# pgriewank/SAMSIM

Hardware: AMD Instinct MI355X
Metric: column-timesteps/sec (higher is better)
Workload: dtype f64

## Files before the change

samsim_amd/csrc/samsim_kernels.hip:

```cpp
#include <hip/hip_runtime.h>
#include <math.h>

#include <type_traits>

#include "samsim_device.h"
#include "samsim_probe.h"
#include "samsim_step_types.h"
#include "samsim_thermo.h"
#include "samsim_surface.h"
#include "samsim_sweeps_fused.h"
#include "samsim_melt.h"
#include "samsim_sweeps_unfused.h"
#include "samsim_regrid.h"
#include "samsim_tracers.h"

namespace {

template <class K>
__device__ RARE void vital_signs(Col &c, const Ctx &x) {
  const samsim_config &g = x.p->cfg;
  const int Na = c.Na;
  double sH = 0.0, sm = 0.0, sS = 0.0, resist = 0.0, sth = 0.0, sS1 = 0.0, sm1 = 0.0;
  for (int k = 1; k <= Na; ++k) {
    const double H_abs = LAY(SAMSIM_A_H_ABS, k), m = LAY(SAMSIM_A_M, k), S_abs = LAY(SAMSIM_A_S_ABS, k);
// ... 96 lines not shown
    if (time > 86400.0 * 25.0) CL(T2m) = 15.0;
    else if (time > 86400.0 * 15.0) CL(T2m) = 1.0;
  } else if (K::general && CFG(testcase) == 9) {
    if (time < 19.75 * 3600.0) CL(T2m) = 0.0;
    else if (time < 86400.0 * 3.0 + 2.25 * 3600.0) CL(T2m) = -15.0;
    else CL(T2m) = 1.0;
  } else if (K::general && CFG(testcase) == 34) {
    if (time < 2.0 * 3600.0) CL(T2m) = 0.0;
    else if (time < 86400.0 * 5.0) CL(T2m) = -15.0;
    else if (time < 86400.0 * 7.0) CL(T2m) = -5.0;
    else CL(T2m) = 1.0;
  } else if (K::general && CFG(testcase) == 6) {
    const double t[8] = {1714.0, 1676.0, 1525.0, 1483.0, 1385.0, 1349.0, 1160.0, 1100.0};
    for (int i = 0; i < 8; ++i) {
      if (time > t[i] * 60.0) { CL(T2m) = (i == 0) ? -19.0 : ((i & 1) ? -5.0 : -18.0); break; }
    }
  }
}

template <class K>
__device__ __forceinline__ void column_step(Col &c, Ctx &x, long long col, double time, int tc, bool out_step, bool next_out,
                                            bool last_step) {
  const samsim_config &g = x.p->cfg;
  const int N = c.N;

  if (out_step) {
    vital_signs<K>(c, x);
    if ((c.flags & COLF_RESTART) && col >= x.out_col0 && col < x.out_col0 + x.out_ncols) {
      const size_t oc = (size_t)(col - x.out_col0), on = (size_t)x.out_ncols;
      for (int k = 1; k <= N; ++k) x.out_lay[((size_t)SAMSIM_A_RAY * N + (k - 1)) * on + oc] = LAY(SAMSIM_A_RAY, k);
    }
  }

  if (CFG(atmoflux_flag) == 2) {
    if (time == time_input(tc)) {
      CL(T2m) = x.f_T2m[x.soff + tc - 1];
      CL(liquid_precip) = x.f_precip[x.soff + tc - 1];
    } else {
      const double temp = (time - time_input(tc - 1)) / (time_input(tc) - time_input(tc - 1));
      CL(T2m) = (1.0 - temp) * x.f_T2m[x.soff + tc - 2] + temp * x.f_T2m[x.soff + tc - 1];
      CL(liquid_precip) = (1.0 - temp) * x.f_precip[x.soff + tc - 2] + temp * x.f_precip[x.soff + tc - 1];
    }
    CL(T2m) = CL(T2m) + GSI(SAMSIM_S_DT2M);
    CL(liquid_precip) = CL(liquid_precip) * GSI(SAMSIM_S_PRECIP_SCALE);
  }

  c.bgc_flood = 0.0; c.bgc_grav = false;
  snow_fall<K>(c, x);
  snow_block<K>(c, x);
  if (c.status) return;

  c.ray_all = (c.flags & COLF_DIRTY) != 0;
  const bool whole_wave = !wave_any(!c.ray_all);
  if (c.ray_all) { ST_COUNT(CT_DIRTY, 1); ST_COUNT(CT_L_DIRTY, (unsigned long long)__popcll(__ballot(1))); sweep_thermo_expulsion<K>(c, x, out_step, whole_wave); }
  else prologue_top_layer<K>(c, x);
  c.flags &= (COLF_REGULAR | COLF_FLUSHED);
  if (c.status) return;

  int Na = c.Na;
  const bool do_grav = (CFG(grav_flag) == 2 && Na > 1), do_beer = (CFG(boundflux_flag) == 2);
  const bool coupling = (CL(m_snow) > 0.0 && CL(thick_snow) < g.thick_min);
  const bool flood_possible = (CFG(flood_flag) > 1 && CL(m_snow) > 0.0 && CFG(freeboard_snow_flag) == 0 &&
                               CL(m_snow) > c.buoy_s * (rho_l - rho_s));
  [[maybe_unused]] const bool fused_col = do_grav && !out_step && (c.step + 1 != 1) && (!flood_possible || (CFG(flood_flag) == 2 && !coupling)) &&
                     !(K::general && CFG(testcase) == 5 && c.step + 1 == 2) && !HAS_BGC &&
                     !(K::general && CFG(prescribe_flag) == 2)
                     && (c.flags & COLF_REGULAR) != 0
      ;
#if SAMSIM_PATH_MODE == 1
  const bool fused = false;
#else
  const bool fused = !wave_any(!fused_col);
#endif

  ST_MARK(ST_PRO);
  ST_COUNT(CT_WAVESTEPS, 1);
  ST_COUNT(CT_LANES, (unsigned long long)__popcll(__ballot(1)));
  ST_COUNT(CT_L_COUPLING, (unsigned long long)__popcll(__ballot(coupling)));
  ST_COUNT(CT_L_FLOODP, (unsigned long long)__popcll(__ballot(flood_possible)));
  ST_COUNT(CT_L_IRREG, (unsigned long long)__popcll(__ballot((c.flags & COLF_REGULAR) == 0)));
  ST_COUNT(CT_L_UNFUSED, (unsigned long long)__popcll(__ballot(!fused_col)));
  bool surface_done = false;
  if (fused) {
    ST_COUNT(CT_FUSED, 1);
    if (flood_possible) {
      ExpelledEnds en;
      sweep_expulsion_transfer<K, true>(c, x, &en);
      THICK_RULE_INIT(tr);
      if (en.psi_gN > 0.0) {
        const double temp2 = en.psi_gN * THICK_AT(tr, Na) * rho_l;
        en.mN = en.mN + temp2;
        en.SN = en.SN + temp2 * x.S_bu_bottom;
        en.HN = en.HN + temp2 * c_l * g.T_bottom;
      }
      const double buoy = c.buoy_s * (rho_l - rho_s) + en.buoy_g * rho_l;
      if (CL(m_snow) > buoy) {
        GS(FREEBOARD) = (buoy - CL(m_snow)) / rho_l;
        if (GS(FREEBOARD) < 0.0) {
          FloodEnds e;
          e.S1 = en.S1; e.H1 = en.H1; e.m1 = en.m1; e.th1 = LAY(SAMSIM_A_THICK, 1);
          e.SN = en.SN; e.HN = en.HN; e.mN = en.mN; e.TN = en.TN;
          const double th1_before = e.th1;
          flood_core<K>(c, x, SPEC(SP_FL_HP), SPEC(SP_FL_SALL), e);
          LAY(SAMSIM_A_THICK, 1) = e.th1;
          refresh_ray_top<K>(c, x, e.th1, en.psi_l1, en.S_br1);
          c.flags |= COLF_FLOODED;
          SPEC(SP_FLD_S1) = e.S1; SPEC(SP_FLD_H1) = e.H1; SPEC(SP_FLD_M1) = e.m1; SPEC(SP_FLD_TH1_BEFORE) = th1_before;
          if (e.deep) { c.flags |= COLF_FLOOD_DEEP; SPEC(SP_FL_HP) = e.incS; SPEC(SP_FL_SALL) = e.incH; }
        }
      }
    }
    testcase_scalars<K>(c, x, g, time);
    const bool late_rad = wave_any(coupling);
    double beer0 = 0.0;
    if (!late_rad) {
      beer0 = radiation_header<K>(c, x, time, tc);
      c.frad = 0.0;
    }
    bool store_default = true, decide_psi = false;
    if (K::fixed && K::boundflux_flag == 2 && K::flush_flag == 5) { store_default = next_out || last_step; decide_psi = true; }
    if (K::fixed && K::flush_flag == 1) store_default = next_out || last_step;
    if (do_beer && !late_rad) sweep_beer<K>(c, x, beer0);
    sweep_down_fused<K>(c, x, store_default, decide_psi, surface_done, coupling, late_rad, time, tc, do_beer);
    ST_MARK(ST_DFUSED);
    if (c.status) return;
  } else {
    ST_COUNT(CT_UNFUSED, 1);
    c.psi_full = true;
    down_unfused<K>(c, x, col, time, tc, out_step, coupling, do_grav, do_beer);
    ST_MARK(ST_DUNFUSED);
    if (c.status) return;
  }

  if (K::general && CFG(tank_flag) == 2) {
    double sS = 0.0, sm = 0.0;
    for (int k = 1; k <= c.Na; ++k) { sS += LAY(SAMSIM_A_S_ABS, k); sm += LAY(SAMSIM_A_M, k); }
    x.S_bu_bottom = (g.S_total - sS) / (g.m_total - sm);
    if (HAS_BGC) {
      double sb = 0.0;
      for (int k = 1; k <= c.Na; ++k) sb += BGC(0, k);
      const double v = (x.bgc_total0 - sb) / (g.m_total - sm);
      for (int t = 0; t < x.n_bgc; ++t) BGC_BOT(t) = v;
    }
  }

  if (!surface_done) surface_flux<K>(c, x);
  ST_MARK(ST_SURF);
  sweep_up_fused<K>(c, x, col, next_out, next_out || last_step);
  ST_MARK(ST_UP);
  if (c.status) return;

  const double melt_thick_snow_old = CL(melt_thick_snow);
  snow_block<K>(c, x);
  if (c.status) return;
  CL(melt_thick_snow) = melt_thick_snow_old + CL(melt_thick_snow);

  bool fb_valid = false;
  if (Na > 1 && CFG(flush_flag) > 2 && (CFG(boundflux_flag) == 2 || (K::general && CFG(boundflux_flag) == 3))) {
    const bool lab = K::general && CFG(boundflux_flag) == 3;
    const double T_surf = lab ? CL(T2m) : CL(T_top);
    const double T_freeze = func_T_freeze(quot(LAY(SAMSIM_A_S_ABS, 1), LAY(SAMSIM_A_M, 1)), CFG(salt_flag), x.tf_c3);
    GS(T_FREEZE) = T_freeze;
    CL(melt_thick) = 0.0;
    const double psi_s1 = LAY(SAMSIM_A_PSI_S, 1);
    if (psi_s1 < psi_s_top_min || T_surf >= T_freeze) {
      if (!c.psi_full) refill_psi_rows<K>(c, x);
      ST_COUNT(CT_L_FREEBOARD, (unsigned long long)__popcll(__ballot(1)));
      GS(FREEBOARD) = func_freeboard<K>(c, x);
      fb_valid = true;
      if (GS(FREEBOARD) > 0.0000000000001) {
        double thick1 = LAY(SAMSIM_A_THICK, 1);
        const double thick1_in = thick1;
        double melt_thick = 0.0;
        sub_melt_thick(LAY(SAMSIM_A_PSI_L, 1), psi_s1, LAY(SAMSIM_A_PSI_G, 1), LAY(SAMSIM_A_T, 1), T_freeze, T_surf, CL(fl_Q1),
                       CL(thick_snow), g.dt, melt_thick, thick1, g.thick_min);
        CL(melt_thick) = melt_thick;
        if (lab) CL(melt_thick) = dmax(CL(melt_thick), 0.0);
        if (CL(thick_snow) >= g.thick_min / 100.0 && CL(melt_thick) > 0.00000000001 && CL(melt_thick_snow) == 0.0) {
          double H_abs = LAY(SAMSIM_A_H_ABS, 1), m = LAY(SAMSIM_A_M, 1);
          const double shift = 1.0 / dmax(GS(PSI_G_SNOW), 0.01) * CL(melt_thick);
          if (shift >= CL(thick_snow)) {
            CL(melt_thick) = CL(melt_thick) - CL(thick_snow) * GS(PSI_G_SNOW);
            H_abs = H_abs + CL(H_abs_snow);
            m = m + CL(m_snow);
// ... 253 lines not shown
```

samsim_amd/csrc/samsim_surface.h:

```cpp
#ifndef SAMSIM_SURFACE_H
#define SAMSIM_SURFACE_H

namespace {

template <class K>
__device__ RARE int snow_coupling_core(Col &c, const Ctx &x, double &H_abs, const double m, const double S_bu, double &T, double &phi) {
  const Salt &s = x.salt;
  double H;
  const double m_snow = CL(m_snow), S_abs_snow = GS(S_ABS_SNOW);
  double phi_sn = GS(PHI_S);
  int rc = 0;
  H_abs = H_abs + m_snow * latent_heat + CL(H_abs_snow);
  CL(H_abs_snow) = -m_snow * latent_heat;
  H = H_abs / m;
#define COUPLE_GETT()                                                                                      \
  do {                                                                                                     \
    double hs = CL(H_abs_snow) / m_snow;                                                                     \
    double T_sn = CL(T_snow);                                                                              \
    rc |= getT(s, hs, S_abs_snow / m_snow, hs / c_l, T_sn, phi_sn);                                        \
    CL(T_snow) = T_sn;                                                                                     \
    rc |= getT(s, H, S_bu, H / c_l, T, phi);                                                               \
  } while (0)
  COUPLE_GETT();
  if (T > 0.0 && H_abs <= -CL(H_abs_snow)) {
// ... 174 lines not shown
      const double temp = (time - time_input(tc - 1)) / (time_input(tc) - time_input(tc - 1));
      CL(fl_sw) = (1.0 - temp) * x.f_sw[x.soff + tc - 2] + temp * x.f_sw[x.soff + tc - 1];
      CL(fl_lw) = (1.0 - temp) * x.f_lw[x.soff + tc - 2] + temp * x.f_lw[x.soff + tc - 1];
    }
  } else if (CFG(atmoflux_flag) == 1) {
    double day = (time + 86400.0 * 180.0) / 86400.0;
    while (day > 360.0) day = day - 360.0;
    const double a = (day - 164.0) / (double)47.9f, b = (day - 206.0) / (double)53.1f;
    CL(fl_sw) = 314.0 * exp(-0.5 * (a * a));
    if (day < 60.0 || day > 300.0) CL(fl_sw) = 0.0;
    GSI(SAMSIM_S_FL_REST) = 118.0 * exp(-0.5 * (b * b)) + 179.0;
  }
  const double pen = (CL(thick_snow) < g.thick_min) ? penetr : 0.0;
  return pen * (1.0 - CL(albedo)) * CL(fl_sw);
}

__device__ __forceinline__ double radiative_T_top(const Col &c, double fl_rest, double T1, double thick_min) {
  double T_old = (CL(thick_snow) < thick_min) ? T1 : CL(T_snow);
  const double emi = (CL(thick_snow) < thick_min) ? emissivity_ice : emissivity_snow;
  const double pen = (CL(thick_snow) < thick_min) ? penetr : 0.0;
  T_old = T_old + zeroK;
  double temp1 = (1.0 - CL(albedo)) * (1.0 - pen) * CL(fl_sw) + fl_rest;
  temp1 = temp1 + emi * 3.0 * sigma * pow_4(T_old);
  temp1 = quot(temp1, emi * 4.0 * sigma * (T_old * T_old * T_old));
  temp1 = temp1 - zeroK;
  T_old = temp1 + zeroK;
  temp1 = (1.0 - CL(albedo)) * (1.0 - pen) * CL(fl_sw) + fl_rest;
  temp1 = temp1 + emi * 3.0 * sigma * pow_4(T_old);
  temp1 = quot(temp1, emi * 4.0 * sigma * (T_old * T_old * T_old));
  temp1 = temp1 - zeroK;
  return temp1;
}

template <class K>
__device__ __forceinline__ void surface_flux(Col &c, const Ctx &x) {
  const samsim_config &g = x.p->cfg;
  const int Na = c.Na;
  const double psi_s1 = LAY(SAMSIM_A_PSI_S, 1), psi_l1 = LAY(SAMSIM_A_PSI_L, 1), psi_g1 = LAY(SAMSIM_A_PSI_G, 1);
  const double thick1 = LAY(SAMSIM_A_THICK, 1), T1 = LAY(SAMSIM_A_T, 1);
  const double k1 = psi_s1 * k_s + psi_l1 * k_l + psi_g1 * 0.0;
  if (CFG(boundflux_flag) == 1) {
    double fl = (T1 - CL(T_top)) / (thick1 / (2.0 * k1));
    if (fabs(fl) > g.max_flux_plate) fl = fl / fabs(fl) * g.max_flux_plate;
    CL(fl_Q1) = fl;
    return;
  }
  if (K::general && CFG(boundflux_flag) == 3) {
    GS(T_FREEZE) = dmin(func_T_freeze(LAY(SAMSIM_A_S_ABS, Na) / LAY(SAMSIM_A_M, Na), CFG(salt_flag), x.tf_c3), 0.0);
    CL(T_top) = T1;
    CL(fl_Q1) = g.alpha_flux_instable * (CL(T_top) - CL(T2m));
    if (CL(fl_Q1) < 0.0) {
      CL(T_top) = dmax(GS(T_FREEZE), T1);
      CL(fl_Q1) = g.alpha_flux_stable * (CL(T_top) - CL(T2m));
    }
    return;
  }
  const double thick_min = g.thick_min;
  const double fl_rest = (!K::general || CFG(atmoflux_flag) == 2) ? CL(fl_lw) + 0.0 + 0.0 : GSI(SAMSIM_S_FL_REST);
  const double emi = (CL(thick_snow) < thick_min) ? emissivity_ice : emissivity_snow;
  const double pen = (CL(thick_snow) < thick_min) ? penetr : 0.0;
  double temp1;
  CL(T_top) = radiative_T_top(c, fl_rest, T1, thick_min);

  double Tf;
  if (CL(thick_snow) >= thick_min / 100.0) Tf = 0.0;
  else Tf = func_T_freeze(quot(LAY(SAMSIM_A_S_ABS, 1), LAY(SAMSIM_A_M, 1)), CFG(salt_flag), x.tf_c3);

  GS(T_FREEZE) = Tf;

  const double k_snow = (CL(thick_snow) >= thick_min / 100.0) ? func_k_snow(CL(m_snow), CL(thick_snow)) : 0.0;
  const double flq_snow_ice = quot(T1 - CL(T_snow), quot(CL(thick_snow), 2.0 * k_snow) + quot(thick1, 2.0 * (psi_s1 * k_s + psi_l1 * k_l)));
  if (CL(T_top) > Tf && Na > 1) {
    temp1 = emi * sigma * pow_4(Tf + zeroK) - (1.0 - CL(albedo)) * (1.0 - pen) * CL(fl_sw) - fl_rest;
    if (CL(thick_snow) >= thick_min) { CL(fl_Q_snow) = temp1; CL(fl_Q1) = flq_snow_ice; }
    else if (CL(thick_snow) >= thick_min / 100.0) { CL(fl_Q_snow) = temp1; CL(fl_Q1) = 0.0; }
    else CL(fl_Q1) = temp1;
    CL(T_top) = Tf;
  } else {
    if (CL(thick_snow) >= thick_min) {
      CL(fl_Q1) = flq_snow_ice;
      CL(fl_Q_snow) = quot(CL(T_snow) - CL(T_top), quot(CL(thick_snow), 2.0 * k_snow));
    } else if (CL(thick_snow) > thick_min / 100.0 && CL(thick_snow) < thick_min) {
      CL(fl_Q1) = 0.0;
      double k = CL(thick_snow) / (CL(thick_snow) + thick1) * k_snow + thick1 / (CL(thick_snow) + thick1) * k1;
      CL(fl_Q_snow) = (CL(T_snow) - CL(T_top)) / ((CL(thick_snow) + thick1) / (2.0 * k));
    } else {
      CL(fl_Q1) = (T1 - CL(T_top)) / (thick1 / (2.0 * k1));
    }
  }
}

__device__ __forceinline__ void sub_melt_thick(double psi_l, double psi_s, double psi_g, double T, double T_freeze, double T_top, double fl_Q,
                               double thick_snow, double dt, double &melt_thick, double &thick, double thick_min) {
  melt_thick = 0.0;
  if (thick_snow < thick_min && T_top >= T_freeze) {
    melt_thick = -fl_Q - 2.0 * (psi_l * k_l + psi_s * k_s) / thick * (T_freeze - T);
    melt_thick = melt_thick * dt / dmax(latent_heat * rho_s * psi_s, 0.000000000000001);
    melt_thick = dmin(psi_l * thick, melt_thick);
  }
  if (psi_s < psi_s_top_min) melt_thick = thick * (1.0 - psi_s / psi_s_top_min);
  if (melt_thick > 0.0 && psi_g > gas_snow_ice2) {
    if (melt_thick > (psi_g - gas_snow_ice2) * thick) {
      melt_thick = melt_thick - (psi_g - gas_snow_ice2) * thick;
      thick = thick * (1.0 - (psi_g - gas_snow_ice2));
    } else {
      thick = thick - melt_thick;
      melt_thick = 0.0;
    }
  }
}

}

#endif
```

samsim_amd/csrc/samsim_sweeps_fused.h:

```cpp
#ifndef SAMSIM_SWEEPS_FUSED_H
#define SAMSIM_SWEEPS_FUSED_H

namespace {


struct RayScan {
  double minp, stp, st;
  double bot, botterm, perm_bot, S_br_bot;
  double buoy_s, min_psi_s;
};
__device__ __forceinline__ void ray_scan_init(RayScan &r) {
  r.minp = 1.0e300; r.stp = 0.0; r.st = 0.0; r.bot = 0.0; r.botterm = 0.0; r.perm_bot = 0.0; r.S_br_bot = 0.0;
  r.buoy_s = 0.0; r.min_psi_s = 1.0e300;
}

struct Expelled { double psi_s, psi_l, psi_g, V_ex; };
__device__ __forceinline__ Expelled expulsion(double phi, double thick, double m, double rth) {
  Expelled e;
  const double V_s = m * phi * (1.0 / rho_s), V_l = m * (1.0 - phi) * (1.0 / rho_l);
  e.V_ex = dmax(V_l + V_s - thick, 0.0);
  e.psi_s = V_s * rth;
  e.psi_l = (V_l - e.V_ex) * rth;
  e.psi_g = (thick - V_l - V_s + e.V_ex) * rth;
  e.psi_l = dmax(e.psi_l, 0.0);
  e.psi_g = dmax(e.psi_g, 0.0);
  return e;
}

template <class K>
__device__ __forceinline__ void s1_layer(Col &c, const Ctx &x, int k, int Na, bool do_ray, double T, double phi, double S_bu,
                                         double m, double thick, double rth, RayScan &r, bool sparse_rows = false, const double *S_br_T = nullptr) {
  const samsim_config &g = x.p->cfg;
  const double S_br = S_br_T ? *S_br_T : S_br_clamped(x.salt, T, S_bu);
  const Expelled e = expulsion(phi, thick, m, rth);
  r.min_psi_s = dmin(r.min_psi_s, e.psi_s);
  r.buoy_s += e.psi_s * thick;
  if (k == 1) c.psi_l_top = e.psi_l;
  if (do_ray) {
    const double perm = x.p17 * pow_3p1(1000.0 * fabs(e.psi_l));
    if (k == Na) {
      r.S_br_bot = S_br;
      r.bot = thick * e.psi_s / psi_s_min;
      r.perm_bot = perm;
      r.botterm = r.bot / perm;
    } else {
      const double height = r.st + r.bot;
      r.minp = dmin(r.minp, perm);
      r.stp = r.stp + quot(thick, perm);
      r.st = r.st + thick;
      double ray;
      const double d_S_br = S_br - r.S_br_bot;
      const bool harmonic = CFG(harmonic_flag) == 2;
      const double h_sum = harmonic ? r.st + r.bot : 0.0, h_den = harmonic ? r.stp + r.botterm : 0.0;
      if (sparse_rows && harmonic && k != 1 && !x.ray_rows_all) {
        constexpr double q_ray = ray_crit * (1.0 - 0x1p-20) * (kappa_l * mu);
        const double P = grav_f * rho_l * bbeta * d_S_br * height * h_sum, Q = q_ray * h_den;
        ST_COUNT(CT_RAY_ROWS, 1);
        if ((__builtin_amdgcn_ballot_w64(!(P < Q)) & __builtin_amdgcn_ballot_w64(!(r.minp < x.p14))) == 0ull) {
          ST_COUNT(CT_RAY_ROWS_BOUND, 1);
          return;
        }
      }
      if (harmonic) {
        const double hp = (r.minp < x.p14) ? 0.0 : quot(h_sum, h_den);
        ray = grav_f * rho_l * bbeta * d_S_br * height * hp;
      } else {
        ray = grav_f * rho_l * bbeta * d_S_br * height * dmin(r.minp, r.perm_bot);
      }
      ray = ray * (1.0 / (kappa_l * mu));
      ray = dmax(ray, 0.0);
      if (!sparse_rows) {
        LAYU(SAMSIM_A_RAY, k) = ray;
      } else if (k == 1 || x.ray_rows_all || wave_any(ray > ray_crit)) {
        LAYU(SAMSIM_A_RAY, k) = ray;
        x.rflag[(k - 1) >> 6] = x.rflag[(k - 1) >> 6] | (1ull << ((k - 1) & 63));
      }
    }
  }
}

template <class K>
__device__ __forceinline__ void flood_handover(Col &c, const Ctx &x, const RayScan &all, const RayScan &below_top, double thick_bottom) {
  const samsim_config &g = x.p->cfg;
  if (!(CFG(flood_flag) > 1 && c.Na > 1 && CL(m_snow) > all.buoy_s * (rho_l - rho_s))) return;
  SPEC(SP_FL_HP) = quot(all.st + all.bot, all.stp + all.botterm);
  SPEC(SP_FL_SALL) = all.st + thick_bottom;
  SPEC(SP_MINP) = below_top.minp; SPEC(SP_STP) = below_top.stp; SPEC(SP_ST) = below_top.st;
  SPEC(SP_BOT) = below_top.bot; SPEC(SP_BOTTERM) = below_top.botterm; SPEC(SP_SBR_BOT) = below_top.S_br_bot;
}

template <class K>
__device__ __forceinline__ void prologue_top_layer(Col &c, const Ctx &x) {
  const samsim_config &g = x.p->cfg;
  const int Na = c.Na;
  const bool do_ray = (CFG(grav_flag) >= 2 && Na > 1);
  RayScan r;
  r.minp = SPEC(SP_MINP); r.stp = SPEC(SP_STP); r.st = SPEC(SP_ST);
  r.bot = SPEC(SP_BOT); r.botterm = SPEC(SP_BOTTERM); r.perm_bot = SPEC(SP_PERM_BOT);
  r.S_br_bot = SPEC(SP_SBR_BOT); r.buoy_s = SPEC(SP_BUOY_S); r.min_psi_s = SPEC(SP_MIN_PSI_S);
  const RayScan r_below_top = r;
  const double H_abs = LAY(SAMSIM_A_H_ABS, 1), m = LAY(SAMSIM_A_M, 1), thick = LAY(SAMSIM_A_THICK, 1);
  double S_abs = LAY(SAMSIM_A_S_ABS, 1);
  if (S_abs < 0.0) { S_abs = 0.0; LAY(SAMSIM_A_S_ABS, 1) = S_abs; }
  double S_bu, H;
  per_mass(S_abs, H_abs, m, S_bu, H);
  if (K::general && CFG(prescribe_flag) == 2) LAY(SAMSIM_A_S_BU, 1) = S_abs / m;
  const double T_test = (Na > 1) ? LAY(SAMSIM_A_T, 2) : g.T_bottom;
  double T, phi = 0.0;
  const int rc = getT_chain(x.salt, H, S_bu, T_test, T, phi);
  LAY(SAMSIM_A_T, 1) = T;
  LAY(SAMSIM_A_PHI, 1) = phi;
  s1_layer<K>(c, x, 1, Na, do_ray, T, phi, S_bu, m, thick, recip(thick), r);
  if (do_ray && CFG(flood_flag) > 1 && CL(m_snow) > r.buoy_s * (rho_l - rho_s)) {
    THICK_RULE_INIT(tr);
    flood_handover<K>(c, x, r, r_below_top, THICK_AT(tr, Na));
  }
  c.neg_psi = r.min_psi_s < 0.0;
  c.buoy_s = r.buoy_s;
  if (rc) STOPC(rc, 1);
}

template <class K>
__device__ RARE void sweep_beer(Col &c, const Ctx &x, double beer0) {
  const samsim_config &g = x.p->cfg;
  const int Na = c.Na;
  if (!wave_any(beer0 != 0.0)) { c.frad = 0.0; return; }
  if ((c.flags & COLF_REGULAR) != 0) {
    const int n0 = __builtin_amdgcn_readfirstlane(Na);
    const bool same = !wave_any(Na != n0);
    const int kend = same ? n0 : wave_max(Na);
    const int b0 = g.n_top, b1 = g.n_top + g.n_middle;
    double temp2 = beer0, frad = 0.0;
#pragma unroll 1
    for (int st = 0; st < 4; ++st) {
      const int klo = st == 0 ? 1 : (st == 1 ? 2 : (st == 2 ? b0 + 1 : b1 + 1));
      const int khi_s = st == 0 ? 1 : (st == 1 ? b0 : (st == 2 ? b1 : kend));
      if (klo > kend) break;
      if (klo > khi_s) continue;
      const int khi = khi_s < kend ? khi_s : kend;
      const double thick = st == 0 ? LAYU(SAMSIM_A_THICK, 1) : (st == 2 ? LAYU(SAMSIM_A_THICK, g.n_top + 1) : g.thick_0);
      const double e = exp(-extinc * thick);
      if (same) {
        const int kmul = khi < kend ? khi : kend - 1;
        for (int k = klo; k <= kmul; ++k) temp2 = temp2 * e;
        if (khi == kend) frad = temp2 - temp2 * e;
// ... 6 lines not shown
      }
    }
    c.frad = frad;
  } else {
    double temp2 = beer0, e = 0.0, th_prev = -1.0;
    for (int k = 1; k <= Na; ++k) {
      const double thick = LAYU(SAMSIM_A_THICK, k);
      if (thick != th_prev) { e = exp(-extinc * thick); th_prev = thick; }
      if (k == Na) c.frad = temp2 - temp2 * e;
      temp2 = temp2 * e;
    }
  }
}

__device__ __forceinline__ double heat_conductance(double psi_s, double psi_l, double rth) {
  return (2.0 * (psi_s * k_s + psi_l * k_l)) * rth;
}
__device__ __forceinline__ double heat_flux_between(double dT, double g_a, double g_b) {
  return quot(dT * (g_a * g_b), g_a + g_b);
}

__device__ __forceinline__ double out_of_row(double v) {
#if defined(__HIP_DEVICE_COMPILE__)
  double r;
  asm volatile("v_mov_b64 %0, %1" : "=v"(r) : "v"(v));
  return r;
#else
  return v;
#endif
}

template <class K>
__device__ __forceinline__ void sweep_down_fused(Col &c, const Ctx &x, bool store_default, bool decide_psi, bool &surface_done,
                                                 bool couple, bool late_rad, double time, int tc, bool do_beer) {
  const samsim_config &g = x.p->cfg;
  const Salt &s = x.salt;
  const int Na = c.Na;
  const double dt = g.dt;
  double heat_loss = 0.0, cum = 0.0, sum_before = 0.0, sum_after = 0.0, minS = 1.0e300;
  double fb_a2 = 0.0, fb_g2 = 0.0;
  int stop_layer = 0;
  bool store_psi = true;
  double g_up = 0.0, flq_up = 0.0;
  double esum = 0.0;

  struct Ld { double T, S_abs, m, H_abs, ray; };
  struct Raw { double T, S_abs, m, S_bu, S_br, H_abs, ray, H; };
  auto load_ld = [&](int j) -> Ld {
    Ld r;
    r.T = LAYU_LD(SAMSIM_A_T, j);
    r.S_abs = LAYU_LD(SAMSIM_A_S_ABS, j);
    r.m = LAYU_LD(SAMSIM_A_M, j);
    r.H_abs = LAYU_LD(SAMSIM_A_H_ABS, j);
    r.ray = (j <= Na - 1 && ray_row_valid(c, x, j)) ? LAYU(SAMSIM_A_RAY, j) : 0.0;
    return r;
  };
  auto finish = [&](const Ld &l, int j) -> Raw {
    Raw r;
    r.T = l.T; r.S_abs = l.S_abs; r.m = l.m; r.H_abs = l.H_abs; r.ray = l.ray;
    per_mass(r.S_abs, r.H_abs, r.m, r.S_bu, r.H);
    r.S_br = S_br_clamped(s, r.T, r.S_bu);
    return r;
  };
  auto S_br_below = [&](const Ld &l) -> double {
    double S_bu, H;
    per_mass(l.S_abs, l.H_abs, l.m, S_bu, H);
    return S_br_clamped(s, l.T, S_bu);
  };
  struct Lay { double T, SA, mA, S_abs, H_abs, m, flup; bool ch; };

  double flm_j = 0.0;
  double T_up = 0.0, S_br_up = 0.0, S_abs_up = 0.0;
  const int N = c.N;
  Raw raw = finish(load_ld(1), 1);
  Ld ahead = load_ld(2), ahead2 = ahead;
  Lay prev = {0, 0, 1, 0, 0, 0, 0, true};
  double flup_pp = 0.0;
  auto layer = [&](const int j, const Ld &below, const double thick, const double rth, auto last_tag, auto first_tag) {
    constexpr bool LAST = decltype(last_tag)::value, FIRST = decltype(first_tag)::value;
    if (!LAST && !FIRST) { ISA_MARK("D_LAYER_A"); }
    double H_abs = raw.H_abs;
    const Expelled ex = expulsion(phi_from_T(s, raw.H, raw.S_bu, raw.S_br), thick, raw.m, rth);
    const double V_ex = ex.V_ex;
    double psi_g = ex.psi_g, m = raw.m, S_abs = raw.S_abs;
    const double T = raw.T, S_br = raw.S_br;
    double flm_next;
    if (j == 1 || psi_g < (double)0.001f) {
      flm_next = (j == 1) ? -V_ex * rho_l : -V_ex * rho_l + flm_j;
    } else {
      flm_next = -dmax((V_ex - psi_g * thick) * rho_l, 0.0);
      psi_g = dmax(quot(psi_g * thick - V_ex, thick), 0.0);
    }
    if (!FIRST) { fb_a2 += ex.psi_s * thick; fb_g2 += psi_g * thick; }
    if (store_psi || j == 1) {
      LAYU(SAMSIM_A_PSI_S, j) = ex.psi_s;
      LAYU(SAMSIM_A_PSI_L, j) = ex.psi_l;
      LAYU(SAMSIM_A_PSI_G, j) = psi_g;
    }
    const bool flooded_here = FIRST && (c.flags & COLF_FLOODED) != 0;
    const double th_l = flooded_here ? LAYU(SAMSIM_A_THICK, 1) : thick;
    const double gj = heat_conductance(ex.psi_s, ex.psi_l, flooded_here ? recip(th_l) : rth);
    const double flq = (j >= 2) ? heat_flux_between(T - prev.T, g_up, gj) : 0.0;
    if (j == 2) c.flq2 = flq;
    m = m + flm_next - flm_j;
    if (flm_next < 0.0) {
      H_abs = H_abs + flm_next * T * c_l;
      S_abs = S_abs + dmax(flm_next * S_br, -S_abs);
    }
    if (flm_j < 0.0) {
      H_abs = H_abs - flm_j * T_up * c_l;
      S_abs = S_abs - dmax(flm_j * S_br_up, -S_abs_up);
    }
    bool ch = LAST || (flm_next < 0.0) || (flm_j < 0.0);
#if SAMSIM_STAMPS == 2
    if (!LAST && !FIRST) {
      ST_COUNT(CT_ROWS, 1);
      if (__ballot(flm_next < 0.0 || flm_j < 0.0) == 0ull) ST_COUNT(CT_ROWS_STILL, 1);
    }
#endif
    const double SA = S_abs, mA = m;
    S_br_up = S_br;
    flm_j = flm_next;
    double Tl = T;
    if (FIRST && couple) {
      double phi1 = LAYU(SAMSIM_A_PHI, 1);
      const double S_bu1 = S_abs / m;
      LAYU(SAMSIM_A_S_BU, 1) = S_bu1;
      const int rcc = snow_coupling_core<K>(c, x, H_abs, m, S_bu1, Tl, phi1);
      LAYU(SAMSIM_A_T, 1) = Tl;
      LAYU(SAMSIM_A_PHI, 1) = phi1;
      if (rcc && !c.status) { c.status = rcc; x.err_step[c.col] = c.step + 1; x.err_layer[c.col] = 1; }
    }
    if (flooded_here) {
      S_abs = SPEC(SP_FLD_S1); H_abs = SPEC(SP_FLD_H1); m = SPEC(SP_FLD_M1);
      ch = true;
      c.flags &= ~COLF_FLOODED;
    }
    if (LAST) {
      if (psi_g > 0.0) {
        const double t2 = psi_g * thick * rho_l;
        m = m + t2;
        S_abs = S_abs + t2 * x.S_bu_bottom;
        H_abs = H_abs + t2 * c_l * g.T_bottom;
      }
      if (c.flags & COLF_FLOOD_DEEP) {
        S_abs = S_abs + SPEC(SP_FL_HP);
        H_abs = H_abs + SPEC(SP_FL_SALL);
        c.flags &= ~COLF_FLOOD_DEEP;
      }
      if (CFG(turb_flag) == 2) {
        const double turb = Turb_A * exp(Turb_B * (-ocean_density<K>(x) + func_density(T, quot(S_abs, m)))) * dt;
        S_abs = S_abs - turb * (S_abs / m - x.S_bu_bottom);
      }
    }
    if (!LAST && !FIRST) { ISA_MARK("D_LAYER_B"); }
    ST_MARK(ST_D_A);
    sum_before += S_abs;
    double flup = cum;
    if (!LAST) {
      const double ray = raw.ray;
      if (ray > ray_crit && S_br > S_br_below(below)) {
        const double psi_s = ex.psi_s;
        if (psi_s > 0.001 && (flooded_here ? quot(S_abs, m) : quot(SA, mA)) > 0.1) {
          ST_COUNT(CT_DRAIN_WAVE, 1);
          ST_COUNT(CT_DRAIN_LANE, (unsigned long long)__popcll(__ballot(1)));
          const double psi_l = ex.psi_l;
          double flux = x_grav * (ray - ray_crit) * dt * th_l;
          flux = dmin(flux, psi_l * rho_l * th_l);
          S_abs = S_abs - flux * S_br;
          if (S_abs < 0.0 && !stop_layer) stop_layer = j;
// ... 3 lines not shown
          cum = cum + flux;
          flup = dmin(cum, psi_l * rho_l * th_l);
          ch = true;
        }
      }
    }
    sum_after += S_abs;
#if defined(__HIP_DEVICE_COMPILE__)
    asm volatile("" : "+v"(sum_before), "+v"(sum_after));
#endif
    if (!LAST && !FIRST) { ISA_MARK("D_LAYER_C"); }
    if (j > 1) {
      if (prev.flup > 0.0) {
        prev.H_abs = prev.H_abs + prev.flup * T * c_l;
        prev.S_abs = prev.S_abs + dmin(prev.flup * S_br_clamped(s, T, quot(SA, mA)), S_abs);
        prev.ch = true;
      }
      if (flup_pp > 0.0) {
        prev.H_abs = prev.H_abs - flup_pp * prev.T * c_l;
        prev.S_abs = prev.S_abs - dmin(flup_pp * S_br_clamped(s, prev.T, quot(prev.SA, prev.mA)), prev.S_abs);
        prev.ch = true;
      }
      if (j - 1 >= 2) {
        const double H_b = prev.H_abs;
        prev.H_abs = prev.H_abs + (flq - flq_up) * dt;
        prev.H_abs = prev.H_abs + c.frad * dt;
        esum += H_b - prev.H_abs;
      }
      if (wave_any(prev.ch)) {
        LAYU(SAMSIM_A_M, j - 1) = prev.m;
        LAYU(SAMSIM_A_S_ABS, j - 1) = prev.S_abs;
      }
      LAYU(SAMSIM_A_H_ABS, j - 1) = prev.H_abs;
      minS = dmin(minS, prev.S_abs);
      flup_pp = prev.flup;
    }
    g_up = gj; flq_up = flq;
    T_up = out_of_row(T); S_abs_up = out_of_row(SA);
    prev.T = FIRST ? out_of_row(Tl) : T_up; prev.SA = S_abs_up; prev.mA = mA; prev.S_abs = out_of_row(S_abs); prev.H_abs = out_of_row(H_abs);
    prev.m = m; prev.flup = flup; prev.ch = ch;
    if (!LAST && !FIRST) { ISA_MARK("D_LAYER_END"); }
    ST_MARK(ST_D_B);
  };
  const int jmax = wave_max(Na);
  auto request = [&](const int j) { ahead2 = load_ld(j + 2 <= N ? j + 2 : N); };
  auto advance = [&](const int j) { raw = finish(ahead, j + 1); ahead = ahead2; };
  const double thick1 = (c.flags & COLF_FLOODED) ? SPEC(SP_FLD_TH1_BEFORE) : LAYU(SAMSIM_A_THICK, 1);
  if (1 < Na) { request(1); layer(1, ahead, thick1, recip(thick1), std::false_type{}, std::true_type{}); advance(1); }
  if (2 < Na) { request(2); layer(2, ahead, g.thick_0, recip(g.thick_0), std::false_type{}, std::false_type{}); advance(2); }
  if (late_rad) {
    const double beer0 = radiation_header<K>(c, x, time, tc);
    c.frad = 0.0;
    if (do_beer) sweep_beer<K>(c, x, beer0);
  }
  if (decide_psi && Na >= 3) {
    surface_flux<K>(c, x);
    surface_done = true;
    const double thick_min = g.thick_min;
    const double Tf = func_T_freeze(quot(LAYU(SAMSIM_A_S_ABS, 1), LAYU(SAMSIM_A_M, 1)), CFG(salt_flag), x.tf_c3);
    bool snow_wet = false;
    if (CL(thick_snow) > 0.0) {
      const double H_new = CL(H_abs_snow) + (CL(fl_Q1) - CL(fl_Q_snow)) * dt;
      snow_wet = !(CL(thick_snow) >= thick_min) || !(H_new / CL(m_snow) <= -latent_heat);
    }
    store_psi = store_default || LAYU(SAMSIM_A_PSI_S, 1) < psi_s_top_min || CL(T_top) >= Tf || snow_wet || CL(melt_thick_snow) > 0.0;
  } else {
    store_psi = store_default || decide_psi;
  }
  c.psi_full = store_psi;
  {
    const int b0 = g.n_top, b1 = g.n_top + g.n_middle;
    Ld ahead3 = ahead;
    auto single = [&](const int j, const double th_s, const double rth_s) {
      ahead2 = load_ld(j + 2 <= N ? j + 2 : N);
      layer(j, ahead, th_s, rth_s, std::false_type{}, std::false_type{});
      raw = finish(ahead, j + 1);
      ahead = ahead2;
    };
    int j = 3;
    for (int stretch = 0; stretch < 3; ++stretch) {
      const int hi_s = stretch == 0 ? b0 : (stretch == 1 ? b1 : N);
      const int hi = hi_s < jmax - 1 ? hi_s : jmax - 1;
      const double th_s = stretch == 1 ? LAYU(SAMSIM_A_THICK, g.n_top + 1) : g.thick_0, rth_s = recip(th_s);
      for (; j + 2 <= hi; j += 3) {
        ISA_MARK("D_ITER_BEGIN");
        ST_MARK(ST_DFUSED);
        if (j + 2 < Na) {
          ST_COUNT(CT_DOWN_TRIPS, 3);
          ahead2 = load_ld(j + 2 <= N ? j + 2 : N);
          layer(j, ahead, th_s, rth_s, std::false_type{}, std::false_type{});
          raw = finish(ahead, j + 1);
          ahead3 = load_ld(j + 3 <= N ? j + 3 : N);
          layer(j + 1, ahead2, th_s, rth_s, std::false_type{}, std::false_type{});
          raw = finish(ahead2, j + 2);
          ahead = load_ld(j + 4 <= N ? j + 4 : N);
          layer(j + 2, ahead3, th_s, rth_s, std::false_type{}, std::false_type{});
          raw = finish(ahead3, j + 3);
        } else if (j < Na) {
          ISA_MARK("D_RARE_BEGIN");
          ST_COUNT(CT_DOWN_TRIPS, 1);
          single(j, th_s, rth_s);
          if (j + 1 < Na) { ST_COUNT(CT_DOWN_TRIPS, 1); single(j + 1, th_s, rth_s); }
        }
        ISA_MARK("D_ITER_END");
      }
      for (; j <= hi; ++j) {
        if (j < Na) single(j, th_s, rth_s);
      }
    }
  }
  const double thick_Na = (Na > g.n_top && Na <= g.n_top + g.n_middle) ? LAYU(SAMSIM_A_THICK, g.n_top + 1) : g.thick_0;
  layer(Na, ahead, thick_Na, recip(thick_Na), std::true_type{}, std::false_type{});
  if (prev.flup > 0.0) {
    prev.H_abs = prev.H_abs + prev.flup * g.T_bottom * c_l;
    prev.S_abs = prev.S_abs + dmin(prev.flup * S_br_clamped(s, g.T_bottom, x.S_bu_bottom), x.S_bu_bottom * 2000.0);
  }
  if (flup_pp > 0.0) {
    prev.H_abs = prev.H_abs - flup_pp * prev.T * c_l;
    prev.S_abs = prev.S_abs - dmin(flup_pp * S_br_clamped(s, prev.T, quot(prev.SA, prev.mA)), prev.S_abs);
  }
  CL(grav_drain) = CL(grav_drain) + prev.flup;
  if (CFG(grav_heat_flag) == 2) prev.H_abs = prev.H_abs + heat_loss - prev.flup * c_l * g.T_bottom;
  {
    const double H_b = prev.H_abs;
    prev.H_abs = prev.H_abs + (c.fl_q_bottom - flq_up) * dt;
    prev.H_abs = prev.H_abs + c.frad * dt;
    c.esum = esum + (H_b - prev.H_abs);
  }
  LAYU(SAMSIM_A_M, Na) = prev.m;
  LAYU(SAMSIM_A_S_ABS, Na) = prev.S_abs;
  LAYU(SAMSIM_A_H_ABS, Na) = prev.H_abs;
  minS = dmin(minS, prev.S_abs);
  if (store_psi) { SPEC(SP_FB_A2) = fb_a2; SPEC(SP_FB_G2) = fb_g2; }
  CL(grav_salt) = CL(grav_salt) + sum_before;
  CL(grav_salt) = CL(grav_salt) - sum_after;
  if (stop_layer) STOPC(21234, stop_layer);
  if (minS < 0.0) STOPC(1337, 0);
}

template <class K>
__device__ __forceinline__ void sweep_up_fused(Col &c, const Ctx &x, long long col, bool next_is_output, bool store_phi) {
  const samsim_config &g = x.p->cfg;
  const Salt &s = x.salt;
  const int Na = c.Na;
  const double dt = g.dt, thick_min = g.thick_min;
  const bool thin_snow = (CL(thick_snow) >= thick_min / 100.0 && CL(thick_snow) < thick_min);
  const bool do_ray = (CFG(grav_flag) >= 2 && Na > 1);
  const bool keep_ray = next_is_output && col >= x.out_col0 && col < x.out_col0 + x.out_ncols;
  const double H_abs_snow_before = CL(H_abs_snow);
  double esum = c.esum;
  double T_test = g.T_bottom;
  int rc = 0, rc_layer = 0;
  RayScan r;
  ray_scan_init(r);
  if (keep_ray) {
    const size_t oc = (size_t)(col - x.out_col0), on = (size_t)x.out_ncols;
    for (int k = 1; k <= c.N - 1; ++k) x.out_lay[((size_t)SAMSIM_A_RAY * c.N + (k - 1)) * on + oc] = LAYU(SAMSIM_A_RAY, k);
  }
  for (int w = 0; w <= (c.N - 1) >> 6; ++w) x.rflag[w] = 0ull;
  __builtin_amdgcn_wave_barrier();
  if (do_ray && Na <= c.N - 1 && x.ray_rows_all) LAYU(SAMSIM_A_RAY, Na) = 0.0;
  struct UL { double th, H, m, S; };
  const bool regular_wave = !wave_any((c.flags & COLF_REGULAR) == 0);
  UL cur, nxt, nn;
  bool alive = true, neg_salt = false;
  NewtonConsts nc_s = newton_consts(s);
  auto body = [&](const int k, const UL &row, const double th_k, const double rth_k, auto top_tag, auto lite_tag) {
    constexpr bool TOP = decltype(top_tag)::value;
    constexpr bool LITE = decltype(lite_tag)::value;
    const double H_k = row.H, m_k = row.m, S_k = row.S;
    double H_abs = H_k;
    const double m = m_k;
    if (TOP) {
      const double flq_below = (Na >= 2) ? c.flq2 : c.fl_q_bottom;
// ... 25 lines not shown
      if (!TOP) { ST_COUNT(CT_ABOVE_ROWS, 1); if (__ballot(evals < 0)) ST_COUNT(CT_ABOVE_FAST, 1); }
      evals &= 0x7fffffff;
      const bool was_odd = (evals >> 30) & 1;
      const int redo = (evals >> 16) & 0x3fff;
      evals &= 0xffff;
      const unsigned long long om = __ballot(was_odd);
      if (om) { ST_COUNT(CT_ODD_LANES, (unsigned long long)__popcll(om)); ST_COUNT(CT_ODD_WAVES, 1); ST_COUNT(CT_ODD_EVALS_WAVE, (unsigned long long)wave_max(redo)); }
    }
    ST_COUNT(CT_UP_TRIPS, 1);
    ST_COUNT(CT_NEWTON_WAVE, (unsigned long long)wave_max(evals));
    { int tot = 0; unsigned long long mk = __ballot(1); while (mk) { const int ln = __ffsll((long long)mk) - 1; tot += __builtin_amdgcn_readlane(evals, ln); mk &= mk - 1; }
      ST_COUNT(CT_NEWTON_LANE, (unsigned long long)tot); }
#else
    int rr = TOP ? getT(s, H, S_bu, T_test, T, phi) : getT_chain<LITE>(s, H, S_bu, T_test, T, phi, nullptr, LITE ? nullptr : &S_br_T, &nc_s);
#endif
    if (!TOP) { ISA_MARK("U_GETT_END"); }
    ST_MARK(ST_U_GETT);
    if (rr && !rc) { rc = rr; rc_layer = k; }
    T_test = T;
    LAYU(SAMSIM_A_T, k) = T;
    if (store_phi || TOP || k >= Na - 1) LAYU(SAMSIM_A_PHI, k) = phi;
    if (!TOP && !LITE) {
      neg_salt = neg_salt || (S_abs < 0.0);
      s1_layer<K>(c, x, k, Na, do_ray, T, phi, S_bu, m, th_k, rth_k, r, true, &S_br_T);
    }
    ST_MARK(ST_U_TAIL);
  };
  const int kmax = wave_max(Na);
  auto load3 = [&](int j) -> UL { UL u; u.th = 0.0; u.H = LAYU_LD(SAMSIM_A_H_ABS, j); u.m = LAYU_LD(SAMSIM_A_M, j); u.S = LAYU_LD(SAMSIM_A_S_ABS, j); return u; };
  auto load4 = [&](int j) -> UL { UL u = load3(j); u.th = LAYU(SAMSIM_A_THICK, j); return u; };
  auto layers = [&](auto lite_tag) {
  if (regular_wave) {
    const int kc = kmax >= 2 ? kmax - 1 : 1;
    UL a = load3(kmax), b = load3(kc), d = b;
    auto one = [&](const int k, const UL &row, UL &req, const double th_s, const double rth_s) {
      req = load3(k >= 3 ? k - 2 : 1);
      if (k <= Na) body(k, row, th_s, rth_s, std::false_type{}, lite_tag);
    };
    const int b0 = g.n_top, b1 = g.n_top + g.n_middle;
    int k = kmax;
    for (int stretch = 0; stretch < 3; ++stretch) {
      const int klo = stretch == 0 ? b1 + 1 : (stretch == 1 ? b0 + 1 : 2);
      const double th_s = stretch == 1 ? LAYU(SAMSIM_A_THICK, g.n_top + 1) : g.thick_0, rth_s = recip(th_s);
      nc_s = newton_consts(s);
      for (; k - 2 >= klo; k -= 3) {
        ISA_MARK("U_ITER_BEGIN");
        ST_MARK(ST_UP);
        one(k, a, d, th_s, rth_s);
        ISA_MARK("U_LAYER_2");
        one(k - 1, b, a, th_s, rth_s);
        ISA_MARK("U_LAYER_3");
        one(k - 2, d, b, th_s, rth_s);
        ISA_MARK("U_ITER_END");
      }
      for (; k >= klo; --k) {
        ISA_MARK("U_REST_BEGIN");
        ST_MARK(ST_UP);
        one(k, a, d, th_s, rth_s);
        a = b; b = d;
        ISA_MARK("U_REST_END");
      }
    }
    cur = a;
  } else {
    cur = load4(Na); nxt = load4(Na >= 2 ? Na - 1 : 1); nn = nxt;
    for (int k = kmax; k >= 2; --k) {
      if (k > Na) continue;
      nn = load4(k >= 3 ? k - 2 : 1);
      body(k, cur, cur.th, recip(cur.th), std::false_type{}, lite_tag);
      cur = nxt; nxt = nn;
    }
  }
  };
  const bool lite = K::fixed && CFG(flush_flag) == 5 && wave_any((c.flags & COLF_FLUSHED) != 0);
  if (lite) { ST_COUNT(CT_LITE, 1); layers(std::true_type{}); } else layers(std::false_type{});
  __builtin_amdgcn_wave_barrier();
  if (neg_salt || lite) c.flags |= COLF_DIRTY;
  body(1, cur, LAYU(SAMSIM_A_THICK, 1), 0.0, std::true_type{}, std::false_type{});
  if (!alive) return;
  if (!lite) {
  SPEC(SP_MINP) = r.minp; SPEC(SP_STP) = r.stp; SPEC(SP_ST) = r.st;
  SPEC(SP_BOT) = r.bot; SPEC(SP_BOTTERM) = r.botterm; SPEC(SP_PERM_BOT) = r.perm_bot;
  SPEC(SP_SBR_BOT) = r.S_br_bot; SPEC(SP_BUOY_S) = r.buoy_s; SPEC(SP_MIN_PSI_S) = r.min_psi_s;
  }
  double bal = esum + (H_abs_snow_before - CL(H_abs_snow));
  bal = bal + (double)Na * (c.frad * dt);
  if (thin_snow || CL(thick_snow) >= thick_min) bal = bal + c.fl_q_bottom * dt - CL(fl_Q_snow) * dt;
  else bal = bal + c.fl_q_bottom * dt - CL(fl_Q1) * dt;
  if (fabs(bal / dt) > 0.00001) STOPC(431, 0);
  if (rc) STOPC(rc, rc_layer);
}

}

#endif
```

Baseline: 778.8 million.

## Hand off top and bottom layer values in registers between prologue and sweeps

The top-layer prologue values (T, S, m, H, thickness, ray) are passed into the fused down-sweep in registers, and the layer-1 porosity and temperature are captured during the down-sweep to feed a new surface_flux_core. The down-sweep's final bottom rows are handed to the up-sweep so it can skip reloading them. This removes redundant global-memory reloads of layer data across stages. In exchange it adds register pressure and several correctness-sensitive conditions (flooded flag, kc mismatch, wave uniformity).

```diff
diff --git a/samsim_amd/csrc/samsim_kernels.hip b/samsim_amd/csrc/samsim_kernels.hip
--- a/samsim_amd/csrc/samsim_kernels.hip
+++ b/samsim_amd/csrc/samsim_kernels.hip
@@ -152,6 +152,7 @@
     }
   }
 
+  ISA_MARK("P_HEAD");
   if (CFG(atmoflux_flag) == 2) {
     if (time == time_input(tc)) {
       CL(T2m) = x.f_T2m[x.soff + tc - 1];
@@ -166,14 +167,18 @@
   }
 
   c.bgc_flood = 0.0; c.bgc_grav = false;
+  ISA_MARK("P_SNOW");
   snow_fall<K>(c, x);
   snow_block<K>(c, x);
   if (c.status) return;
 
+  ISA_MARK("P_PROLOGUE");
   c.ray_all = (c.flags & COLF_DIRTY) != 0;
   const bool whole_wave = !wave_any(!c.ray_all);
+  const bool top_handed = !wave_any(c.ray_all);
+  TopHand top = {0.0, 0.0, 0.0, 0.0, 0.0, 0.0};
   if (c.ray_all) { ST_COUNT(CT_DIRTY, 1); ST_COUNT(CT_L_DIRTY, (unsigned long long)__popcll(__ballot(1))); sweep_thermo_expulsion<K>(c, x, out_step, whole_wave); }
-  else prologue_top_layer<K>(c, x);
+  else prologue_top_layer<K>(c, x, top);
   c.flags &= (COLF_REGULAR | COLF_FLUSHED);
   if (c.status) return;
 
@@ -201,6 +206,7 @@
   ST_COUNT(CT_L_IRREG, (unsigned long long)__popcll(__ballot((c.flags & COLF_REGULAR) == 0)));
   ST_COUNT(CT_L_UNFUSED, (unsigned long long)__popcll(__ballot(!fused_col)));
   bool surface_done = false;
+  BottomHand bot = {0.0, 0.0, 0.0, 0.0, 0.0, 0.0, 0};
   if (fused) {
     ST_COUNT(CT_FUSED, 1);
     if (flood_possible) {
@@ -241,7 +247,7 @@
     if (K::fixed && K::boundflux_flag == 2 && K::flush_flag == 5) { store_default = next_out || last_step; decide_psi = true; }
     if (K::fixed && K::flush_flag == 1) store_default = next_out || last_step;
     if (do_beer && !late_rad) sweep_beer<K>(c, x, beer0);
-    sweep_down_fused<K>(c, x, store_default, decide_psi, surface_done, coupling, late_rad, time, tc, do_beer);
+    sweep_down_fused<K>(c, x, store_default, decide_psi, surface_done, coupling, late_rad, time, tc, do_beer, top_handed, top, bot);
     ST_MARK(ST_DFUSED);
     if (c.status) return;
   } else {
@@ -266,10 +272,12 @@
 
   if (!surface_done) surface_flux<K>(c, x);
   ST_MARK(ST_SURF);
-  sweep_up_fused<K>(c, x, col, next_out, next_out || last_step);
+  ISA_MARK("P_UP_ENTRY");
+  sweep_up_fused<K>(c, x, col, next_out, next_out || last_step, fused, bot);
   ST_MARK(ST_UP);
   if (c.status) return;
 
+  ISA_MARK("P_POST");
   const double melt_thick_snow_old = CL(melt_thick_snow);
   snow_block<K>(c, x);
   if (c.status) return;
diff --git a/samsim_amd/csrc/samsim_surface.h b/samsim_amd/csrc/samsim_surface.h
--- a/samsim_amd/csrc/samsim_surface.h
+++ b/samsim_amd/csrc/samsim_surface.h
@@ -230,12 +230,11 @@
   return temp1;
 }
 
-template <class K>
-__device__ __forceinline__ void surface_flux(Col &c, const Ctx &x) {
+template <class K, class TF>
+__device__ __forceinline__ void surface_flux_core(Col &c, const Ctx &x, const double psi_s1, const double psi_l1, const double psi_g1,
+                                                  const double thick1, const double T1, TF Tf_top) {
   const samsim_config &g = x.p->cfg;
   const int Na = c.Na;
-  const double psi_s1 = LAY(SAMSIM_A_PSI_S, 1), psi_l1 = LAY(SAMSIM_A_PSI_L, 1), psi_g1 = LAY(SAMSIM_A_PSI_G, 1);
-  const double thick1 = LAY(SAMSIM_A_THICK, 1), T1 = LAY(SAMSIM_A_T, 1);
   const double k1 = psi_s1 * k_s + psi_l1 * k_l + psi_g1 * 0.0;
   if (CFG(boundflux_flag) == 1) {
     double fl = (T1 - CL(T_top)) / (thick1 / (2.0 * k1));
@@ -262,7 +261,7 @@
 
   double Tf;
   if (CL(thick_snow) >= thick_min / 100.0) Tf = 0.0;
-  else Tf = func_T_freeze(quot(LAY(SAMSIM_A_S_ABS, 1), LAY(SAMSIM_A_M, 1)), CFG(salt_flag), x.tf_c3);
+  else Tf = Tf_top();
 
   GS(T_FREEZE) = Tf;
 
@@ -287,6 +286,14 @@
     }
   }
 }
+template <class K>
+__device__ __forceinline__ void surface_flux(Col &c, const Ctx &x) {
+  const samsim_config &g = x.p->cfg;
+  const double psi_s1 = LAY(SAMSIM_A_PSI_S, 1), psi_l1 = LAY(SAMSIM_A_PSI_L, 1), psi_g1 = LAY(SAMSIM_A_PSI_G, 1);
+  const double thick1 = LAY(SAMSIM_A_THICK, 1), T1 = LAY(SAMSIM_A_T, 1);
+  surface_flux_core<K>(c, x, psi_s1, psi_l1, psi_g1, thick1, T1,
+                       [&]() { return func_T_freeze(quot(LAY(SAMSIM_A_S_ABS, 1), LAY(SAMSIM_A_M, 1)), CFG(salt_flag), x.tf_c3); });
+}
 
 __device__ __forceinline__ void sub_melt_thick(double psi_l, double psi_s, double psi_g, double T, double T_freeze, double T_top, double fl_Q,
                                double thick_snow, double dt, double &melt_thick, double &thick, double thick_min) {
diff --git a/samsim_amd/csrc/samsim_sweeps_fused.h b/samsim_amd/csrc/samsim_sweeps_fused.h
--- a/samsim_amd/csrc/samsim_sweeps_fused.h
+++ b/samsim_amd/csrc/samsim_sweeps_fused.h
@@ -29,7 +29,8 @@
 
 template <class K>
 __device__ __forceinline__ void s1_layer(Col &c, const Ctx &x, int k, int Na, bool do_ray, double T, double phi, double S_bu,
-                                         double m, double thick, double rth, RayScan &r, bool sparse_rows = false, const double *S_br_T = nullptr) {
+                                         double m, double thick, double rth, RayScan &r, bool sparse_rows = false, const double *S_br_T = nullptr,
+                                         double *ray_out = nullptr) {
   const samsim_config &g = x.p->cfg;
   const double S_br = S_br_T ? *S_br_T : S_br_clamped(x.salt, T, S_bu);
   const Expelled e = expulsion(phi, thick, m, rth);
@@ -71,6 +72,7 @@
       ray = dmax(ray, 0.0);
       if (!sparse_rows) {
         LAYU(SAMSIM_A_RAY, k) = ray;
+        if (ray_out) *ray_out = ray;
       } else if (k == 1 || x.ray_rows_all || wave_any(ray > ray_crit)) {
         LAYU(SAMSIM_A_RAY, k) = ray;
         x.rflag[(k - 1) >> 6] = x.rflag[(k - 1) >> 6] | (1ull << ((k - 1) & 63));
@@ -89,8 +91,11 @@
   SPEC(SP_BOT) = below_top.bot; SPEC(SP_BOTTERM) = below_top.botterm; SPEC(SP_SBR_BOT) = below_top.S_br_bot;
 }
 
+struct TopHand { double T, S_abs, m, H_abs, thick, ray; };
+struct BottomHand { double H, m, S, bH, bm, bS; int kc; };
+
 template <class K>
-__device__ __forceinline__ void prologue_top_layer(Col &c, const Ctx &x) {
+__device__ __forceinline__ void prologue_top_layer(Col &c, const Ctx &x, TopHand &top) {
   const samsim_config &g = x.p->cfg;
   const int Na = c.Na;
   const bool do_ray = (CFG(grav_flag) >= 2 && Na > 1);
@@ -110,7 +115,8 @@
   const int rc = getT_chain(x.salt, H, S_bu, T_test, T, phi);
   LAY(SAMSIM_A_T, 1) = T;
   LAY(SAMSIM_A_PHI, 1) = phi;
-  s1_layer<K>(c, x, 1, Na, do_ray, T, phi, S_bu, m, thick, recip(thick), r);
+  top.T = T; top.S_abs = S_abs; top.m = m; top.H_abs = H_abs; top.thick = thick; top.ray = 0.0;
+  s1_layer<K>(c, x, 1, Na, do_ray, T, phi, S_bu, m, thick, recip(thick), r, false, nullptr, &top.ray);
   if (do_ray && CFG(flood_flag) > 1 && CL(m_snow) > r.buoy_s * (rho_l - rho_s)) {
     THICK_RULE_INIT(tr);
     flood_handover<K>(c, x, r, r_below_top, THICK_AT(tr, Na));
@@ -183,7 +189,8 @@
 
 template <class K>
 __device__ __forceinline__ void sweep_down_fused(Col &c, const Ctx &x, bool store_default, bool decide_psi, bool &surface_done,
-                                                 bool couple, bool late_rad, double time, int tc, bool do_beer) {
+                                                 bool couple, bool late_rad, double time, int tc, bool do_beer,
+                                                 bool top_handed, const TopHand &top, BottomHand &bot) {
   const samsim_config &g = x.p->cfg;
   const Salt &s = x.salt;
   const int Na = c.Na;
@@ -223,10 +230,19 @@
   double flm_j = 0.0;
   double T_up = 0.0, S_br_up = 0.0, S_abs_up = 0.0;
   const int N = c.N;
-  Raw raw = finish(load_ld(1), 1);
-  Ld ahead = load_ld(2), ahead2 = ahead;
+  ISA_MARK("P_DOWN_ENTRY");
+  Ld ahead = load_ld(2), ahead2 = {0.0, 0.0, 0.0, 0.0, 0.0};
+  Ld first;
+  if (top_handed) {
+    first.T = top.T; first.S_abs = top.S_abs; first.m = top.m; first.H_abs = top.H_abs;
+    first.ray = (c.flags & COLF_FLOODED) ? LAYU(SAMSIM_A_RAY, 1) : top.ray;
+  } else {
+    first = load_ld(1);
+  }
+  Raw raw = finish(first, 1);
   Lay prev = {0, 0, 1, 0, 0, 0, 0, true};
   double flup_pp = 0.0;
+  double t1_psi_s = 0.0, t1_psi_l = 0.0, t1_psi_g = 0.0, t1_T = 0.0, t1_th = 0.0, t1_m = 0.0, done_S = 0.0;
   auto layer = [&](const int j, const Ld &below, const double thick, const double rth, auto last_tag, auto first_tag) {
     constexpr bool LAST = decltype(last_tag)::value, FIRST = decltype(first_tag)::value;
     if (!LAST && !FIRST) { ISA_MARK("D_LAYER_A"); }
@@ -287,6 +303,7 @@
       ch = true;
       c.flags &= ~COLF_FLOODED;
     }
+    if (FIRST) { t1_psi_s = ex.psi_s; t1_psi_l = ex.psi_l; t1_psi_g = psi_g; t1_T = Tl; t1_th = th_l; t1_m = m; }
     if (LAST) {
       if (psi_g > 0.0) {
         const double t2 = psi_g * thick * rho_l;
@@ -356,6 +373,7 @@
         LAYU(SAMSIM_A_S_ABS, j - 1) = prev.S_abs;
       }
       LAYU(SAMSIM_A_H_ABS, j - 1) = prev.H_abs;
+      done_S = prev.S_abs;
       minS = dmin(minS, prev.S_abs);
       flup_pp = prev.flup;
     }
@@ -369,25 +387,26 @@
   const int jmax = wave_max(Na);
   auto request = [&](const int j) { ahead2 = load_ld(j + 2 <= N ? j + 2 : N); };
   auto advance = [&](const int j) { raw = finish(ahead, j + 1); ahead = ahead2; };
-  const double thick1 = (c.flags & COLF_FLOODED) ? SPEC(SP_FLD_TH1_BEFORE) : LAYU(SAMSIM_A_THICK, 1);
+  const double thick1 = (c.flags & COLF_FLOODED) ? SPEC(SP_FLD_TH1_BEFORE) : (top_handed ? top.thick : LAYU(SAMSIM_A_THICK, 1));
   if (1 < Na) { request(1); layer(1, ahead, thick1, recip(thick1), std::false_type{}, std::true_type{}); advance(1); }
   if (2 < Na) { request(2); layer(2, ahead, g.thick_0, recip(g.thick_0), std::false_type{}, std::false_type{}); advance(2); }
+  ISA_MARK("P_DOWN_AFTER2");
   if (late_rad) {
     const double beer0 = radiation_header<K>(c, x, time, tc);
     c.frad = 0.0;
     if (do_beer) sweep_beer<K>(c, x, beer0);
   }
   if (decide_psi && Na >= 3) {
-    surface_flux<K>(c, x);
+    const double Tf = func_T_freeze(quot(done_S, t1_m), CFG(salt_flag), x.tf_c3);
+    surface_flux_core<K>(c, x, t1_psi_s, t1_psi_l, t1_psi_g, t1_th, t1_T, [&]() { return Tf; });
     surface_done = true;
     const double thick_min = g.thick_min;
-    const double Tf = func_T_freeze(quot(LAYU(SAMSIM_A_S_ABS, 1), LAYU(SAMSIM_A_M, 1)), CFG(salt_flag), x.tf_c3);
     bool snow_wet = false;
     if (CL(thick_snow) > 0.0) {
       const double H_new = CL(H_abs_snow) + (CL(fl_Q1) - CL(fl_Q_snow)) * dt;
       snow_wet = !(CL(thick_snow) >= thick_min) || !(H_new / CL(m_snow) <= -latent_heat);
     }
-    store_psi = store_default || LAYU(SAMSIM_A_PSI_S, 1) < psi_s_top_min || CL(T_top) >= Tf || snow_wet || CL(melt_thick_snow) > 0.0;
+    store_psi = store_default || t1_psi_s < psi_s_top_min || CL(T_top) >= Tf || snow_wet || CL(melt_thick_snow) > 0.0;
   } else {
     store_psi = store_default || decide_psi;
   }
@@ -433,6 +452,7 @@
       }
     }
   }
+  ISA_MARK("P_DOWN_EXIT");
   const double thick_Na = (Na > g.n_top && Na <= g.n_top + g.n_middle) ? LAYU(SAMSIM_A_THICK, g.n_top + 1) : g.thick_0;
   layer(Na, ahead, thick_Na, recip(thick_Na), std::true_type{}, std::false_type{});
   if (prev.flup > 0.0) {
@@ -454,6 +474,9 @@
   LAYU(SAMSIM_A_M, Na) = prev.m;
   LAYU(SAMSIM_A_S_ABS, Na) = prev.S_abs;
   LAYU(SAMSIM_A_H_ABS, Na) = prev.H_abs;
+  bot.H = prev.H_abs; bot.m = prev.m; bot.S = prev.S_abs;
+  bot.kc = jmax - 1;
+  bot.bH = LAYU_LD(SAMSIM_A_H_ABS, bot.kc); bot.bm = LAYU_LD(SAMSIM_A_M, bot.kc); bot.bS = LAYU_LD(SAMSIM_A_S_ABS, bot.kc);
   minS = dmin(minS, prev.S_abs);
   if (store_psi) { SPEC(SP_FB_A2) = fb_a2; SPEC(SP_FB_G2) = fb_g2; }
   CL(grav_salt) = CL(grav_salt) + sum_before;
@@ -463,7 +486,8 @@
 }
 
 template <class K>
-__device__ __forceinline__ void sweep_up_fused(Col &c, const Ctx &x, long long col, bool next_is_output, bool store_phi) {
+__device__ __forceinline__ void sweep_up_fused(Col &c, const Ctx &x, long long col, bool next_is_output, bool store_phi,
+                                               bool bottom_handed, const BottomHand &bot) {
   const samsim_config &g = x.p->cfg;
   const Salt &s = x.salt;
   const int Na = c.Na;
@@ -555,7 +579,14 @@
   auto layers = [&](auto lite_tag) {
   if (regular_wave) {
     const int kc = kmax >= 2 ? kmax - 1 : 1;
-    UL a = load3(kmax), b = load3(kc), d = b;
+    UL a, b;
+    if (bottom_handed) {
+      a.th = 0.0; a.H = bot.H; a.m = bot.m; a.S = bot.S;
+      if (bot.kc == kc) { b.th = 0.0; b.H = bot.bH; b.m = bot.bm; b.S = bot.bS; } else b = load3(kc);
+    } else {
+      a = load3(kmax); b = load3(kc);
+    }
+    UL d = {0.0, 0.0, 0.0, 0.0};
     auto one = [&](const int k, const UL &row, UL &req, const double th_s, const double rth_s) {
       req = load3(k >= 3 ? k - 2 : 1);
       if (k <= Na) body(k, row, th_s, rth_s, std::false_type{}, lite_tag);
@@ -598,6 +629,7 @@
   const bool lite = K::fixed && CFG(flush_flag) == 5 && wave_any((c.flags & COLF_FLUSHED) != 0);
   if (lite) { ST_COUNT(CT_LITE, 1); layers(std::true_type{}); } else layers(std::false_type{});
   __builtin_amdgcn_wave_barrier();
+  ISA_MARK("P_UP_TOP");
   if (neg_salt || lite) c.flags |= COLF_DIRTY;
   body(1, cur, LAYU(SAMSIM_A_THICK, 1), 0.0, std::true_type{}, std::false_type{});
   if (!alive) return;
```

Result: no change. 783.6 million, median of 6 (+0.6%).
